# randomwons/RayTracingStudy

Measured on AMD Instinct MI355X. Metric: Mrays/s (primary+shadow) at 1920x1080, 64 spp, 100000 spheres, higher is better.
Workload: dtype f32; 1 GPU; c3: 64 spp Monte-Carlo accumulate, ~100k spheres (headline); width=1920, height=1080, spp=64, n_spheres=100000, octree_depth=7, octree_nodes=37384, prim_refs=153448, leaf_capacity=12, parallelism=single, frames_in_flight=1, rays_per_frame=184963628, primary_per_frame=132710400

## Files before the change

raytracingstudy_amd/csrc/rt_bins.h:

```cpp
#pragma once
#include <hip/hip_runtime.h>

#include "rt_bins_math.h"
#include "rt_params.h"
#include "rt_walk.h"

namespace rtamd {

typedef uint32_t bin_u32x8 __attribute__((ext_vector_type(8)));
typedef uint32_t bin_u32x2 __attribute__((ext_vector_type(2)));
typedef __attribute__((address_space(4))) const bin_u32x8 BinEntries;

struct BinBest {
    float t;
    uint32_t idx, ref;
};

__device__ __forceinline__ bool bin_entry(const bin_u32x8 e, float o0, float o1, float o2, float d0,
                                          float d1, float d2, BinBest& best) {
    if (!__any(best.t >= __uint_as_float(e[7]))) return false;
    const float4 sp = make_float4(__uint_as_float(e[0]), __uint_as_float(e[1]), __uint_as_float(e[2]),
                                  __uint_as_float(e[3]));
    float th;
    if (isect(o0, o1, o2, d0, d1, d2, sp, 0.0f, INFINITY, th)) {
        if (th < best.t || (th == best.t && e[4] < best.idx)) {
            best.t = th;
            best.idx = e[4];
            best.ref = e[5];
        }
    }
    return true;
}

__device__ __forceinline__ bool bin_nearest(uint2 hdr, unsigned long long word, bool active, float o0,
                                            float o1, float o2, float d0, float d1, float d2,
                                            float& tout, uint32_t& iout) {
    KernArgs* ka = kernargs();
    BinBest best{active ? INFINITY : -INFINITY, kNoHit, kNoHit};
    BinEntries* ent = reinterpret_cast<BinEntries*>(reinterpret_cast<uintptr_t>(ka->bin_ent)) + hdr.x;
    while (word) {
        const uint32_t k = static_cast<uint32_t>(__builtin_ctzll(word));
        word &= word - 1ull;
        if (!bin_entry(ent[k], o0, o1, o2, d0, d1, d2, best)) break;
    }
    const uint32_t nw = *reinterpret_cast<__attribute__((address_space(4))) const uint32_t*>(
        reinterpret_cast<uintptr_t>(ka->bin_info + kBinInfoWide));
    if (nw) {
        BinEntries* wide = reinterpret_cast<BinEntries*>(reinterpret_cast<uintptr_t>(ka->bin_wide));
        for (uint32_t k = 0; k < nw; ++k)
            if (!bin_entry(wide[k], o0, o1, o2, d0, d1, d2, best)) break;
    }
    if (best.ref == kNoHit) return false;
    tout = best.t;
    iout = best.ref;
    return true;
}

__device__ __forceinline__ bool bin_header(uint32_t tox, uint32_t toy, uint32_t ltw, uint32_t lth,
                                           uint2& hdr, unsigned long long& word) {
    KernArgs* ka = kernargs();
    const uint32_t flag = *reinterpret_cast<__attribute__((address_space(4))) const uint32_t*>(
        reinterpret_cast<uintptr_t>(ka->bin_info + kBinInfoFlag));
    word = 0ull;
    if (tox >= ka->W || toy >= ka->H) {
        hdr = make_uint2(0u, 0u);
        return flag != 0u;
    }
    const uint32_t b = (toy >> kBinShift) * ka->bin_nbx + (tox >> kBinShift);
    const bin_u32x2 h = *reinterpret_cast<__attribute__((address_space(4))) const bin_u32x2*>(
        reinterpret_cast<uintptr_t>(ka->bin_hdr + b));
    const size_t wi = (static_cast<size_t>(b) << (2u * kBinShift - ltw - lth)) + bin_tile_index_log2(tox, toy, ltw, lth);
    const bin_u32x2 w = *reinterpret_cast<__attribute__((address_space(4))) const bin_u32x2*>(
        reinterpret_cast<uintptr_t>(ka->bin_hdr + ka->bin_nb + wi));
    hdr = make_uint2(h.x, h.y);
    if (h.y) word = (static_cast<unsigned long long>(w.y) << 32) | w.x;
    return flag != 0u || h.y == kBinWalk;
}

}
```

raytracingstudy_amd/csrc/rt_bins_host.cpp:

```cpp
#include "rt_frame_math.h"
#include "rt_host.h"

using namespace rtamd;

namespace {

bool bins_gate(rt_renderer* r, const FrameArgs& a, const FramePlan& plan) {
    ScreenBinState& s = r->bins;
    if (r->cfg.flags & RT_FLAG_NO_BINS) return s.last_reason = RT_BINS_OFF_FLAG, false;
    if (a.count_work || !plan.inst.w8() ||
        static_cast<uint64_t>(a.W) * a.H * a.spp < s.min_samples)
        return s.last_reason = RT_BINS_OFF_KERNEL, false;
    float B[9];
    if (!bins_camera_ok(a.cam.K, a.cam.R, a.cam.o) || !cam8_basis(a.cam.K, a.cam.R, a.W, a.H, B))
        return s.last_reason = RT_BINS_OFF_CAMERA, false;
    if (bin_dense_skip_step(s.cadence, r->scene_gen, s.mirror[kBinInfoFrame], s.mirror[kBinInfoFlag]))
        return s.last_reason = RT_BINS_OFF_DENSE, false;
    return true;
}

int bins_buffers(rt_renderer* r, const FrameArgs& a, uint32_t nb, hipStream_t st) {
    ScreenBinState& s = r->bins;
    int ost;
    bool stale;
    if ((ost = s.first_ref.query(r, std::max(1u, r->n_spheres), r->scene_gen, nullptr, 0, &stale))) return ost;
    if (stale) {
        hipError_t e = launch_first_refs(a.sc.prim_sp, a.sc.prim_idx, r->prim_slots, r->d_spheres.p,
                                         r->n_spheres, s.first_ref.buf.p, st);
        if (e != hipSuccess) return hip_fail(r, e, "screen bins (first references)");
        s.first_ref.commit(r->scene_gen, nullptr, 0);
    }
    const size_t want = bin_entries_wanted(s.capacity_test, r->n_spheres, s.mirror[kBinInfoFrame],
                                           s.mirror[kBinInfoFlag], s.mirror[kBinInfoEntries],
                                           s.cadence.last_frame, s.ent.n);
    if (s.ent.n < 2 * want) {
        if (s.ent.p) RT_HIP(r, hipDeviceSynchronize());
        if ((ost = ensure(r, s.ent, 2 * want))) return ost;
    }
    if ((ost = ensure(r, s.rects, std::max(1u, r->n_spheres))) ||
        (ost = ensure(r, s.cnt, 2ull * nb + 1ull)) || (ost = ensure(r, s.offs, nb + 1ull)) ||
        (ost = ensure(r, s.hdr, size_t(nb) * (1u + kBinCap))) ||
        (ost = ensure(r, s.wide, 2ull * kBinWideCap)) || (ost = ensure(r, s.info, kBinInfoWords)))
        return ost;
    if (s.temp_items < nb + 1u || !s.temp.p) {
        const size_t bytes = bins_scan_temp_bytes(nb + 1u);
        if (!bytes) return fail(r, RT_E_HIP, "screen bins: scan scratch size");
        if ((ost = ensure(r, s.temp, bytes))) return ost;
        s.temp_items = nb + 1u;
    }
    return RT_OK;
}

BinBuild bins_build_args(const rt_renderer* r, const FrameArgs& a, const FramePlan& plan, uint32_t nbx,
                         uint32_t nby) {
    const ScreenBinState& s = r->bins;
    const uint32_t nb = nbx * nby;
    BinBuild b{};
    b.spheres = r->d_spheres.p;
    b.first_ref = s.first_ref.buf.p;
    b.n_spheres = r->n_spheres;
    memcpy(b.K, a.cam.K, sizeof(b.K));
    memcpy(b.R, a.cam.R, sizeof(b.R));
    memcpy(b.o, a.cam.o, sizeof(b.o));
    b.W = a.W;
    b.H = a.H;
    b.nbx = nbx;
    b.nby = nby;
    b.tw = plan.grid.tw;
    b.th = plan.grid.th;
    b.shrink = s.shrink;
    b.capacity = static_cast<uint32_t>(s.ent.n / 2);
    b.cap = s.cap;
    b.mean_max = s.mean_max;
    b.frame_id = a.frame_id;
    b.rects = s.rects.p;
    b.counts = s.cnt.p;
    b.cursor = s.cnt.p + nb + 1u;
    b.offs = s.offs.p;
    b.hdr = s.hdr.p;
    b.ent = s.ent.p;
    b.tiles = reinterpret_cast<unsigned long long*>(s.hdr.p + nb);
    b.wide = s.wide.p;
    b.info = s.info.p;
    b.mirror = s.mirror_dev;
    b.temp = s.temp.p;
    b.temp_bytes = s.temp.n;
    return b;
}

int bins_launch(rt_renderer* r, FrameArgs& a, const BinBuild& b, hipStream_t st) {
    ScreenBinState& s = r->bins;
    if (s.timing) RT_HIP(r, hipEventRecord(s.e0, st));
    hipError_t e = launch_screen_bins(b, st);
    if (e != hipSuccess) return hip_fail(r, e, "screen bins");
    if (s.timing) {
        RT_HIP(r, hipEventRecord(s.e1, st));
        s.timed = true;
    }
    s.last_reason = RT_BINS_ON;
    s.cadence.last_frame = a.frame_id;
    s.last_capacity = b.capacity;
    s.nbx = b.nbx;
    s.nby = b.nby;
    s.tw = b.tw;
    s.th = b.th;
    a.bin_hdr = s.hdr.p;
    a.bin_ent = s.ent.p;
    a.bin_nb = b.nbx * b.nby;
    a.bin_wide = s.wide.p;
    a.bin_info = s.info.p;
    a.bin_nbx = b.nbx;
    return RT_OK;
}

}

int rtamd::screen_bins(rt_renderer* r, FrameArgs& a, const FramePlan& plan, hipStream_t st) {
    a.bin_hdr = nullptr;
    a.bin_ent = nullptr;
    a.bin_nb = 0;
    a.bin_wide = nullptr;
    a.bin_info = nullptr;
    a.bin_nbx = 0;
    r->bins.timed = false;
    if (!bins_gate(r, a, plan)) return RT_OK;
    const uint32_t nbx = (a.W + kBinSide - 1u) / kBinSide, nby = (a.H + kBinSide - 1u) / kBinSide;
    if (const int ost = bins_buffers(r, a, nbx * nby, st)) return ost;
    return bins_launch(r, a, bins_build_args(r, a, plan, nbx, nby), st);
}

extern "C" {

int rt_get_bin_info(rt_renderer* r, rt_bin_info* info) {
// ... 71 lines not shown
```

raytracingstudy_amd/csrc/rt_bins_math.h:

```cpp
#pragma once
#include <math.h>
#include <stddef.h>
#include <stdint.h>

#if defined(__HIPCC__)
#define RT_BINS_HD __host__ __device__
#else
#define RT_BINS_HD
#endif

namespace rtamd {

constexpr uint32_t kBinShift = 3;
constexpr uint32_t kBinSide = 1u << kBinShift;
constexpr uint32_t kBinCap = 64;
constexpr uint32_t kBinWalk = 0xFFFFFFFFu;
constexpr uint32_t kBinWideCap = 32;
constexpr uint32_t kBinMeanMax = 48;
constexpr uint32_t kBinDenseSkip = 15;
constexpr uint64_t kBinMinSamples = 1ull << 22;

constexpr double kBinSlackDist = 1.0 / 131072.0;
constexpr double kBinSlackPix = 1.0 / 64.0;
constexpr double kBinSlackPixRel = 1e-6;
// ... 79 lines not shown
    return ((y & (kBinSide - 1u)) / th) * (kBinSide / tw) + (x & (kBinSide - 1u)) / tw;
}

RT_BINS_HD inline uint32_t bin_tile_index_log2(uint32_t x, uint32_t y, uint32_t ltw, uint32_t lth) {
    return (((y & (kBinSide - 1u)) >> lth) << (kBinShift - ltw)) + ((x & (kBinSide - 1u)) >> ltw);
}

RT_BINS_HD inline bool bin_rect_overlaps_tile(uint32_t rect, uint32_t tile, uint32_t tw, uint32_t th) {
    const uint32_t per_row = kBinSide / tw;
    const uint32_t tx0 = (tile % per_row) * tw, ty0 = (tile / per_row) * th;
    const uint32_t tx1 = tx0 + tw - 1u, ty1 = ty0 + th - 1u;
    return !((rect & 15u) > tx1 || ((rect >> 4) & 15u) < tx0 || ((rect >> 8) & 15u) > ty1 ||
             ((rect >> 12) & 15u) < ty0);
}

RT_BINS_HD inline uint64_t bin_tile_word(const uint32_t* rects, uint32_t cnt, uint32_t tile, uint32_t tw,
                                         uint32_t th) {
    uint64_t w = 0;
    for (uint32_t k = 0; k < cnt && k < 64u; ++k)
        if (bin_rect_overlaps_tile(rects[k], tile, tw, th)) w |= uint64_t(1) << k;
    return w;
}

enum BinInfoWord : uint32_t {
    kBinInfoFlag = 0,
    kBinInfoWide,
    kBinInfoEntries,
    kBinInfoNonEmpty,
    kBinInfoLongest,
    kBinInfoOver,
    kBinInfoFrame,
    kBinInfoWords = 8
};
constexpr uint32_t kBinFlagCapacity = 1u;
constexpr uint32_t kBinFlagWide = 2u;
constexpr uint32_t kBinFlagDense = 4u;

struct BinCadence {
    uint32_t skip = 0;
    uint64_t gen = 0;
    uint32_t last_frame = 0;
};

inline bool bin_dense_skip_step(BinCadence& c, uint64_t scene_gen, uint32_t mirror_frame,
                                uint32_t mirror_flag) {
    if (c.gen != scene_gen) c.skip = 0, c.gen = scene_gen;
    if (!c.skip && c.last_frame && mirror_frame == c.last_frame && mirror_flag == kBinFlagDense) {
        c.skip = kBinDenseSkip;
        c.last_frame = 0;
    }
    if (!c.skip) return false;
    --c.skip;
    return true;
}

inline size_t bin_entries_wanted(uint32_t capacity_test, uint32_t n_spheres, uint32_t mirror_frame,
// ... 13 lines not shown
```

raytracingstudy_amd/csrc/rt_host.h:

```cpp
#pragma once
#include <hip/hip_runtime.h>
#include <math.h>
#include <stdio.h>
#include <string.h>

#include <algorithm>
#include <chrono>
#include <string>
#include <vector>

#include "../../include/rt.h"
#include "octree_gpu.h"
#include "rt_bins_math.h"
#include "rt_overlap_math.h"
#include "rt_params.h"
#include "scene_build.h"

struct ncclComm;

namespace rtamd {

hipError_t launch_scene(const FrameArgs& a, const FramePlan& plan, hipStream_t st);
bool variant_available(uint32_t v);
hipError_t launch_compat(const FrameArgs& a, hipStream_t st);
// ... 13 lines not shown
hipError_t launch_multihit(const FrameArgs& a, const void* rays, void* hits, void* counts, uint32_t n,
                           uint32_t k, unsigned long long* counters, hipStream_t st);
hipError_t launch_overlap(const FrameArgs& a, const void* probes, void* indices, void* counts,
                          uint32_t n, uint32_t k, bool skip_self, float slack_m,
                          unsigned long long* counters, hipStream_t st);
hipError_t launch_gbuffer(const FrameArgs& a, void* hits, void* normals, void* albedo,
                          unsigned long long* counters, hipStream_t st);

struct BinBuild {
    const float4* spheres;
    const uint32_t* first_ref;
    uint32_t n_spheres;
    float K[9], R[9], o[3];
    uint32_t W, H, nbx, nby;
    uint32_t tw, th;
    double shrink;
    uint32_t capacity;
    uint32_t cap;
    uint32_t mean_max;
    uint32_t frame_id;
    uint4* rects;
    uint32_t* counts;
    uint32_t* cursor;
    uint32_t* offs;
    uint2* hdr;
    uint4* ent;
    unsigned long long* tiles;
    uint4* wide;
    uint32_t* info;
    uint32_t* mirror;
    void* temp;
    size_t temp_bytes;
};
hipError_t launch_first_refs(const float4* prim_sp, const uint32_t* prim_idx, uint32_t n_slots,
                             const float4* spheres, uint32_t n_spheres, uint32_t* first_ref,
                             hipStream_t st);
size_t bins_scan_temp_bytes(uint32_t n_items);
hipError_t launch_screen_bins(const BinBuild& b, hipStream_t st);

extern thread_local std::string g_last_error;
int fail(rt_renderer* r, int code, const std::string& msg);
int hip_fail(rt_renderer* r, hipError_t e, const char* what);

#define RT_HIP(r, call)                                   \
    do {                                                  \
        hipError_t e_ = (call);                           \
        if (e_ != hipSuccess) return hip_fail((r), e_, #call); \
    } while (0)

template <typename T>
struct DevBuf {
    T* p = nullptr;
// ... 50 lines not shown
    void* recv[F] = {nullptr, nullptr};
    std::vector<hipEvent_t> rendered[F], sent[F];
    hipEvent_t recvd[F] = {nullptr, nullptr}, unpacked[F] = {nullptr, nullptr}, out_ready = nullptr;
    bool used[F] = {false, false};
    bool timing = false;
    bool timed[F] = {false, false};
    std::vector<hipEvent_t> t_start[F], t_end[F];
    hipEvent_t t_unpacked[F] = {nullptr, nullptr};
    uint64_t frame = 0;
    bool broken = false;
    enum Fault { kNone = 0, kCreate, kComm, kSlab, kQueue };
    int fault = kNone;
    uint32_t fault_k = 0;
    uint32_t W = 0, H = 0, S = 0;
    size_t slab_bytes = 0;
    std::vector<std::vector<uint32_t>> ids;
    std::vector<uint32_t> all_ids;
    uint32_t* d_all_ids = nullptr;
};

struct ScreenBinState {
    DerivedRecords<uint32_t> first_ref;
    DevBuf<uint4> rects, ent, wide;
    DevBuf<uint32_t> cnt, offs, info;
    DevBuf<uint2> hdr;
    uint32_t tw = 1, th = 1;
    DevBuf<unsigned char> temp;
    uint32_t temp_items = 0;
    uint32_t* mirror = nullptr;
    uint32_t* mirror_dev = nullptr;
    uint32_t cap = 64, capacity_test = 0, mean_max = 48;
    double shrink = 1.0;
    uint64_t min_samples = kBinMinSamples;
    BinCadence cadence;
    uint32_t last_reason = RT_BINS_NO_FRAME;
    uint32_t last_capacity = 0, nbx = 0, nby = 0;
    hipEvent_t e0 = nullptr, e1 = nullptr;
    bool timing = false, timed = false;
    void release() {
        first_ref.buf.release();
        rects.release();
        ent.release();
        wide.release();
        cnt.release();
        offs.release();
        info.release();
        hdr.release();
        temp.release();
        if (e0) (void)hipEventDestroy(e0);
        if (e1) (void)hipEventDestroy(e1);
        if (mirror) (void)hipHostFree(mirror);
    }
};

struct QueryScratch {
    DevBuf<unsigned long long> counters;
    DevBuf<float4> ray;
    DevBuf<uint2> hit;
    DevBuf<uint2> multi_hits;
    DevBuf<uint32_t> multi_count;
    DevBuf<float4> probe;
    DevBuf<uint32_t> overlap_idx;
    DevBuf<uint32_t> overlap_count;
    void release() {
        counters.release();
        ray.release();
        hit.release();
        multi_hits.release();
        multi_count.release();
// ... 140 lines not shown
```

raytracingstudy_amd/csrc/rt_kernels.hip:

```cpp
#include <hip/hip_runtime.h>

#include <algorithm>
#include <mutex>
#include <vector>

#include "rt_params.h"
#include "rt_shade.h"
#include "rt_sorted.h"

namespace rtamd {

__device__ __forceinline__ unsigned long long wave_sum(unsigned long long v) {
#pragma unroll
    for (int off = 32; off > 0; off >>= 1) v += __shfl_xor(v, off, 64);
    return v;
}

__device__ __forceinline__ void flush_counters(const FrameArgs& a, uint32_t prim, uint32_t shadow,
                                               uint32_t nodes, uint32_t prims) {
    const unsigned long long s0 = prim;
    const unsigned long long s1 = shadow;
    const unsigned long long s2 = wave_sum(nodes);
    const unsigned long long s3 = wave_sum(prims);
    if ((threadIdx.x & 63u) == 0) {
        unsigned long long* c = a.counters + kStatLineBase + (blockIdx.x & 7u) * kStatLineStride;
        atomicAdd(c + 0, s0);
        atomicAdd(c + 1, s1);
        atomicAdd(c + 2, s2);
        atomicAdd(c + 3, s3);
    }
}

template <class C>
__device__ __forceinline__ void scene_body(FrameArgs a) {
    constexpr bool kTiles = C::tiles, kStats = C::stats, kWaveQ = C::waveq, kSort = C::sorted;
    extern __shared__ __attribute__((aligned(16))) float4 lds[];
    float4* acc = lds;
    const uint32_t wave = threadIdx.x >> 6;
    void* stk = reinterpret_cast<uint2*>(lds + (kSort ? 0u : kBlockThreads)) + threadIdx.x;
    float* wl = kSort ? reinterpret_cast<float*>(reinterpret_cast<uint2*>(lds) +
                                                 stack_levels(a.sc, true) * kBlockThreads) +
                            wave * (kSortWaveBytes / 4u)
                      : nullptr;
    const uint32_t lbs = __builtin_amdgcn_readfirstlane(leaf_buf_base(a.sc, kSort));
    if (blockIdx.x == 0) {
        KernArgs* kz = kernargs();
        for (uint32_t i = threadIdx.x; i < kz->ctr_next_words; i += kBlockThreads) kz->ctr_next[i] = 0ull;
    }
    const uint32_t tw = a.tw, th = a.th;
    uint32_t n_shadow = 0, n_nodes = 0, n_prims = 0, n_primary = 0;
#ifdef RT_BLOCK_STATS
    uint32_t bs[2 * kBlockStats] = {};
#else
    uint32_t* bs = nullptr;
#endif
#ifdef RT_TIMELINE
    const unsigned long long tl_start = wall_clock64();
    unsigned long long tl_empty = 0, tl_units = 0;
#endif
    if (kWaveQ) {
        const uint32_t gw = kTiles ? a.tile_size / tw : (a.W + tw - 1) / tw;
        const uint32_t gh = kTiles ? a.tile_size / th : (a.H + th - 1) / th;
        const uint32_t nbx = (gw + 7u) / 8u, nby = (gh + 7u) / 8u;
        const uint32_t nsx = (nbx + 7u) / 8u, nsy = (nby + 7u) / 8u;
        const uint32_t sb_grid = nsx * nsy;
        const uint32_t n_sb = kTiles ? a.n_tiles * sb_grid : sb_grid;
        const uint32_t q = blockIdx.x & 7u;
// ... 77 lines not shown
                if (kTiles) {
                    const uint32_t tile = a.tiles[k];
                    const uint32_t ts = a.tile_size;
                    tox = (tile % a.tiles_x) * ts;
                    toy = (tile / a.tiles_x) * ts;
                    obase = k * ts * ts - toy * ts - tox;
                }
            }
            for (uint32_t cur = w0; cur < w0 + chunk; ++cur) {
                const uint32_t b = cur >> 6, w = cur & 63u;
                const uint32_t wx = sx0 + (b & 7u) * 8u + (w & 7u);
                const uint32_t wy = sy0 + (b >> 3) * 8u + (w >> 3);
                if (wx >= gw || wy >= gh) continue;
                const uint32_t olx = wx * tw, oly = wy * th;
                const uint32_t ox = olx + tox, oy = oly + toy;
#ifdef RT_TIMELINE
                const unsigned long long tu0 = wall_clock64();
#endif
                if (kSort)
                    shade_pixel_sorted<C>(a, wl, stk, ox, oy, obase, n_primary, n_shadow, n_nodes,
                                          n_prims, bs);
                else
                    shade_wave_tile<C>(a, acc, stk, ox, oy, obase, n_primary, n_shadow, n_nodes,
                                       n_prims, bs, lbs);
#ifdef RT_TIMELINE
                const uint32_t sbt = k * sb_grid + (wy >> 6) * nsx + (wx >> 6);
                const unsigned long long uid = (unsigned long long)sbt * 4096u +
                                               (((wy >> 3) & 7u) * 8u + ((wx >> 3) & 7u)) * 64u +
                                               (wy & 7u) * 8u + (wx & 7u);
                if (a.timeline && (threadIdx.x & 63u) == 0 && uid < (1ull << 22)) {
                    const unsigned hw = __builtin_amdgcn_s_getreg((31 << 11) | 4);
                    const unsigned xcc = __builtin_amdgcn_s_getreg((3 << 11) | 20);
                    a.timeline[4ull * 65536 + 3 * uid] = tu0;
                    a.timeline[4ull * 65536 + 3 * uid + 1] = wall_clock64();
                    a.timeline[4ull * 65536 + 3 * uid + 2] =
                        ((unsigned long long)hw << 32) | (xcc << 16) | (blockIdx.x * 4u + wave);
                }
#endif
            }
        }
    } else {
        __shared__ uint32_t tile_slot;
        const uint32_t bts = a.bts;
        const uint32_t wtx = bts / tw, wtiles = wtx * (bts / th);
        const uint32_t per_tile = kTiles ? (a.tile_size / bts) * (a.tile_size / bts) : 0u;
        const uint32_t bx_n = (a.W + bts - 1) / bts;
        const uint32_t n_bt = kTiles ? a.n_tiles * per_tile : bx_n * ((a.H + bts - 1) / bts);
// ... 185 lines not shown
```

raytracingstudy_amd/csrc/rt_shade.h:

```cpp
#pragma once
#include <hip/hip_runtime.h>

#include "rt_params.h"
#include "rt_walk.h"
#include "rt_bins.h"

namespace rtamd {

__device__ __forceinline__ float sat(float x) { return x > 0.0f ? (x < 1.0f ? x : 1.0f) : 0.0f; }

__device__ __forceinline__ uint32_t mix32(uint32_t x) {
    x ^= x >> 16;
    x *= 0x7feb352du;
    x ^= x >> 15;
    x *= 0x846ca68bu;
    x ^= x >> 16;
    return x;
}

__device__ __forceinline__ float u01(uint32_t x) {
    return static_cast<float>(x >> 8) * (1.0f / 16777216.0f);
}

__device__ __forceinline__ void get_ray(const CamArgs& c, float u, float v, float& wx, float& wy,
// ... 8 lines not shown
    wx /= len;
    wy /= len;
    wz /= len;
}


struct PixelOut {
    float r, g, b;
};

__device__ __forceinline__ uint32_t pack_rgba8(const PixelOut& p) {
    const uint32_t r = static_cast<uint32_t>(sat(p.r) * 255.0f);
    const uint32_t g = static_cast<uint32_t>(sat(p.g) * 255.0f);
    const uint32_t b = static_cast<uint32_t>(sat(p.b) * 255.0f);
    return r | (g << 8) | (b << 16) | (255u << 24);
}

template <class C>
__device__ __forceinline__ PixelOut sample_color_unified(const FrameArgs& a, uint32_t x,
                                                         uint32_t y, uint32_t hp, uint32_t s,
                                                         bool valid, uint32_t& n_shadow,
                                                         uint32_t& n_nodes, uint32_t& n_prims,
                                                         void* stk, uint32_t* bs, uint32_t lbs,
                                                         uint32_t tox = 0, uint32_t toy = 0) {
    constexpr bool kStats = C::stats, kCam8 = C::cam8, kOcc = C::occ, kBin = C::bin;
    const SceneArgs& S = a.sc;
    KernArgs* ka = kernargs();
    float u = static_cast<float>(x), v = static_cast<float>(y);
    if (ka->jitter) {
        u = u + u01(mix32(hp ^ (s << 1)));
        v = v + u01(mix32(hp ^ ((s << 1) | 1u)));
    }
    float r0 = ka->cam.o[0], r1 = ka->cam.o[1], r2 = ka->cam.o[2];
    float d0, d1, d2;
    {
        CamArgs cam;
        for (int i = 0; i < 9; ++i) cam.K[i] = ka->cam.K[i], cam.R[i] = ka->cam.R[i];
        get_ray(cam, u, v, d0, d1, d2);
    }
    const float miss_g = sat(d1), miss_b = sat(d2);
    bool active = valid, hit0 = false;
    float lam = 0.0f;
    uint32_t al = 0;
    uint2 occ_hdr = make_uint2(0u, 0u);
#pragma unroll
    for (int phase = 0; phase < 2; ++phase) {
        float t = 0.0f;
        uint32_t idx = 0;
        bool hit = false;
        bool binned = false;
        if (kBin && phase == 0) {
            uint2 bh;
            unsigned long long bw;
            binned = !bin_header(tox, toy, static_cast<uint32_t>(__builtin_ctz(kernargs()->tw)),
                                 static_cast<uint32_t>(__builtin_ctz(kernargs()->th)), bh, bw);
            if (binned) hit = bin_nearest(bh, bw, active, r0, r1, r2, d0, d1, d2, t, idx);
        }
        if (active && !binned) {
            RT_BS(kBsPhase);
            if (phase) RT_BS(kBsPhaseShadow);
            if (phase == 0)
                hit = walk<FramePrimary<kStats, kCam8>>(S, r0, r1, r2, d0, d1, d2, 0.0f, INFINITY, t, idx,
                                                        n_nodes, n_prims, static_cast<uint2*>(stk),
                                                        false, bs, lbs);
            else if (kOcc) {
                hit = shadow_occluded<false>(S, occ_hdr, true, r0, r1, r2, static_cast<uint2*>(stk));
            } else {
                KernArgs* kl = kernargs();
                hit = walk<FrameShadow<kStats>>(
                    S, r0, r1, r2, kl->L[0], kl->L[1], kl->L[2], 0.0f, INFINITY, t, idx, n_nodes,
                    n_prims, static_cast<uint2*>(stk), true, bs);
            }
        }
        if (phase == 0) {
            hit0 = active && hit;
            bool want_shadow = false;
            KernArgs* kb = kernargs();
            if (hit0) {
                RT_BS(kBsShadeLoad);
                RT_BS(kBsShadeLoad);
                const float4 sp = kb->sc.prim_sp[idx];
                const float p0 = r0 + t * d0;
                const float p1 = r1 + t * d1;
                const float p2 = r2 + t * d2;
                const float ir = 1.0f / sp.w;
                const float n0 = (p0 - sp.x) * ir;
                const float n1 = (p1 - sp.y) * ir;
                const float n2 = (p2 - sp.z) * ir;
                const float ndl = n0 * kb->L[0] + n1 * kb->L[1] + n2 * kb->L[2];
                lam = ndl > 0.0f ? ndl : 0.0f;
                want_shadow = ndl > 0.0f && kb->shadows;
                al = kb->sc.prim_al[idx];
                if (kOcc && want_shadow) occ_hdr = kb->sc.prim_occ[idx];
                r0 = p0 + n0 * kShadowEps;
                r1 = p1 + n1 * kShadowEps;
                r2 = p2 + n2 * kShadowEps;
                d0 = kb->L[0];
                d1 = kb->L[1];
                d2 = kb->L[2];
            }
            active = want_shadow;
            n_shadow += static_cast<uint32_t>(__popcll(__ballot(active)));
            if (!__any(active)) break;
        } else if (active && hit) {
            lam = 0.0f;
        }
    }
    PixelOut c{200.0f / 255.0f, miss_g, miss_b};
    if (hit0) {
        const float amb = kernargs()->ambient;
        const float f = amb + (1.0f - amb) * lam;
        c.r = static_cast<float>(al & 0xFFu) * (1.0f / 255.0f) * f;
        c.g = static_cast<float>((al >> 8) & 0xFFu) * (1.0f / 255.0f) * f;
        c.b = static_cast<float>((al >> 16) & 0xFFu) * (1.0f / 255.0f) * f;
    }
    return c;
}

template <class C>
__device__ __forceinline__ void shade_wave_tile(const FrameArgs& a, float4* acc, void* stk,
                                                uint32_t ox, uint32_t oy, uint32_t obase,
                                                uint32_t& n_primary,
                                                uint32_t& n_shadow, uint32_t& n_nodes,
                                                uint32_t& n_prims, uint32_t* bs, uint32_t lbs) {
    constexpr bool kTiles = C::tiles, kProg = C::prog;
    const uint32_t lane = threadIdx.x & 63u;
    const uint32_t spw = a.spw, g = a.g;
    const uint32_t pix = lane / g, sub = lane & (g - 1u);
    const uint32_t qx = pix % a.tw, qy = pix / a.tw;
    const uint32_t x = ox + qx, y = oy + qy;
    const bool lane_pix = pix < a.ppw && x < a.W && y < a.H;
    const bool leader = lane_pix && sub == 0;
    const uint32_t pid = y * a.W + x;
    const uint32_t hp = mix32(a.seedmix ^ pid);
    if (kProg && a.accum_in && leader) acc[threadIdx.x] = a.accum[(size_t)y * a.W + x];
    const uint32_t s_base = kProg ? a.s_base : 0u;
    const uint32_t sub_base = s_base + sub;
    const uint32_t s_end = s_base + a.spp;
    const bool lane_ok = lane_pix && sub < spw;
    for (uint32_t r = 0; r < a.rounds; ++r) {
        const uint32_t sg = r * spw + sub_base;
        const bool valid = lane_ok && sg < s_end;
        n_primary += static_cast<uint32_t>(__popcll(__ballot(valid)));
        PixelOut c = sample_color_unified<C>(a, x, y, hp, sg, valid, n_shadow, n_nodes, n_prims, stk,
                                             bs, lbs, ox, oy);
        if (!valid) c = PixelOut{0.0f, 0.0f, 0.0f};
        for (uint32_t m = 1; m < g; m <<= 1) {
            c.r += __shfl_xor(c.r, static_cast<int>(m), 64);
            c.g += __shfl_xor(c.g, static_cast<int>(m), 64);
            c.b += __shfl_xor(c.b, static_cast<int>(m), 64);
        }
        if (leader) {
            if (r || (kProg && a.accum_in)) {
                const float4 A = acc[threadIdx.x];
                c.r = A.x + c.r;
                c.g = A.y + c.g;
                c.b = A.z + c.b;
            }
            acc[threadIdx.x] = make_float4(c.r, c.g, c.b, 0.0f);
        }
    }
    KernArgs* ko = kernargs();
    if (leader) {
        const float4 A = acc[threadIdx.x];
        if (kProg) ko->accum[(size_t)y * ko->W + x] = A;
        const float isp = ko->inv_spp;
        const PixelOut p{A.x * isp, A.y * isp, A.z * isp};
        const uint32_t rgba = pack_rgba8(p);
// ... 13 lines not shown
```

raytracingstudy_amd/csrc/rt_sorted.h:

```cpp
#pragma once
#include "rt_shade.h"

namespace rtamd {



__device__ __forceinline__ uint32_t jitter_cell(uint32_t hp, uint32_t sg) {
    const uint32_t qu = mix32(hp ^ (sg << 1)) >> (32u - kSortCellBits);
    const uint32_t qv = mix32(hp ^ ((sg << 1) | 1u)) >> (32u - kSortCellBits);
    uint32_t c = 0;
#pragma unroll
    for (uint32_t b = 0; b < kSortCellBits; ++b)
        c |= (((qu >> b) & 1u) << (2u * b)) | (((qv >> b) & 1u) << (2u * b + 1u));
    return c;
}

__device__ __forceinline__ void sample_dir(uint32_t x, uint32_t y, uint32_t hp, uint32_t sg,
                                           float& d0, float& d1, float& d2) {
    KernArgs* ka = kernargs();
    float u = static_cast<float>(x), v = static_cast<float>(y);
    if (ka->jitter) {
        u = u + u01(mix32(hp ^ (sg << 1)));
        v = v + u01(mix32(hp ^ ((sg << 1) | 1u)));
    }
// ... 62 lines not shown
    }
    for (uint32_t j = 0; j < R; ++j) {
        const uint32_t sl = 64u * j + lane;
        if (sl < n) {
            const uint32_t kp = slot[sl].x;
            ord[bcnt[kp >> 8] + (kp & 0xFFu)] = static_cast<uint8_t>(sl);
        }
    }
    uint32_t nl = 0;
    for (uint32_t r = 0; r < R; ++r) {
        const uint32_t i = 64u * r + lane;
        const bool valid = i < n;
        const uint32_t sl = valid ? static_cast<uint32_t>(ord[i]) : 0u;
        n_primary += static_cast<uint32_t>(__popcll(__ballot(valid)));
        float d0, d1, d2;
        sample_dir(x, y, hp, s_base + sl, d0, d1, d2);
        float t = 0.0f;
        uint32_t idx = 0;
        bool hit = false;
        bool binned = false;
        if (kBin) {
            uint2 bh;
            unsigned long long bw;
            binned = !bin_header(x, y, 0u, 0u, bh, bw);
            if (binned) {
                KernArgs* kc = kernargs();
                hit = bin_nearest(bh, bw, valid, kc->cam.o[0], kc->cam.o[1], kc->cam.o[2], d0, d1, d2, t,
                                  idx);
            }
        }
        if (valid && !binned) {
            RT_BS(kBsPhase);
            KernArgs* kc = kernargs();
            hit = walk<SortedPrimary<kStats>>(S, kc->cam.o[0], kc->cam.o[1], kc->cam.o[2], d0, d1, d2,
                                              0.0f, INFINITY, t, idx, n_nodes, n_prims,
                                              static_cast<uint2*>(stk), false, bs);
        }
        bool is_lit = false;
        if (valid) {
            uint2 sv = make_uint2(__float_as_uint(sat(d1)), __float_as_uint(sat(d2)));
            uint8_t kd = 0;
            if (hit) {
                const HitShade h = hit_shade(d0, d1, d2, t, idx, bs);
                is_lit = h.ndl > 0.0f && kernargs()->shadows;
                if (is_lit) {
                    sv = make_uint2(__float_as_uint(t), idx);
                    kd = 2;
                } else {
                    RT_BS(kBsShadeLoad);
                    sv = make_uint2(__float_as_uint(h.ndl > 0.0f ? h.ndl : 0.0f),
                                    kernargs()->sc.prim_al[idx]);
// ... 104 lines not shown
```

raytracingstudy_amd/csrc/screen_bins.hip:

```cpp
#include <hipcub/hipcub.hpp>

#include "rt_bins_math.h"
#include "rt_host.h"

namespace rtamd {

namespace {

__global__ void __launch_bounds__(kBlockThreads)
    first_ref_kernel(const float4* __restrict__ prim_sp, const uint32_t* __restrict__ prim_idx,
                     uint32_t n_slots, const float4* __restrict__ spheres, uint32_t n_spheres,
                     uint32_t* __restrict__ first_ref) {
    const uint32_t i = blockIdx.x * kBlockThreads + threadIdx.x;
    if (i >= n_slots) return;
    const uint32_t k = prim_idx[i];
    if (k >= n_spheres) return;
    const float4 a = prim_sp[i], b = spheres[k];
    if (__float_as_uint(a.x) != __float_as_uint(b.x) || __float_as_uint(a.y) != __float_as_uint(b.y) ||
        __float_as_uint(a.z) != __float_as_uint(b.z) || __float_as_uint(a.w) != __float_as_uint(b.w))
        return;
    atomicMin(first_ref + k, i);
}

struct BinCam {
// ... 16 lines not shown
    const uint32_t ref = first_ref[i];
    BinRect rc;
    rc.cls = kBinDropped;
    const float4 s = spheres[i];
    if (ref != kNoHit) rc = rect_of(s, cam, W, H, shrink);
    rects[i] = make_uint4(rc.x0 | (rc.x1 << 16), rc.y0 | (rc.y1 << 16), __float_as_uint(rc.near_t), rc.cls);
    if (rc.cls == kBinWide) {
        const uint32_t k = atomicAdd(info + kBinInfoWide, 1u);
        if (k < kBinWideCap) {
            wide[2u * k] = make_uint4(__float_as_uint(s.x), __float_as_uint(s.y), __float_as_uint(s.z),
                                      __float_as_uint(s.w));
            wide[2u * k + 1u] = make_uint4(i, ref, 0u | (7u << 4) | (0u << 8) | (7u << 12), __float_as_uint(rc.near_t));
        }
    } else if (rc.cls == kBinBinned) {
        for (uint32_t by = rc.y0 >> kBinShift; by <= (rc.y1 >> kBinShift); ++by)
            for (uint32_t bx = rc.x0 >> kBinShift; bx <= (rc.x1 >> kBinShift); ++bx)
                atomicAdd(counts + by * nbx + bx, 1u);
    }
}

__global__ void __launch_bounds__(kBlockThreads)
    bins_decide_kernel(const uint32_t* __restrict__ counts, const uint32_t* __restrict__ offs, uint32_t nb,
                       uint32_t capacity, uint32_t cap, uint32_t mean_max, uint32_t frame_id,
                       uint32_t* __restrict__ info, uint32_t* __restrict__ mirror) {
    __shared__ uint32_t s_ne[kBlockThreads], s_mx[kBlockThreads], s_ov[kBlockThreads];
    uint32_t ne = 0, mx = 0, ov = 0;
    for (uint32_t b = threadIdx.x; b < nb; b += kBlockThreads) {
        const uint32_t c = counts[b];
        ne += c ? 1u : 0u;
        mx = max(mx, c);
        ov += c > cap ? 1u : 0u;
    }
    s_ne[threadIdx.x] = ne;
    s_mx[threadIdx.x] = mx;
    s_ov[threadIdx.x] = ov;
    __syncthreads();
    for (uint32_t d = kBlockThreads / 2; d > 0; d >>= 1) {
        if (threadIdx.x < d) {
            s_ne[threadIdx.x] += s_ne[threadIdx.x + d];
            s_mx[threadIdx.x] = max(s_mx[threadIdx.x], s_mx[threadIdx.x + d]);
            s_ov[threadIdx.x] += s_ov[threadIdx.x + d];
        }
        __syncthreads();
    }
    if (threadIdx.x == 0) {
        const uint32_t total = offs[nb], nw = info[kBinInfoWide];
        uint32_t flag = 0u;
        if (total > capacity) flag |= kBinFlagCapacity;
        if (nw > kBinWideCap) flag |= kBinFlagWide;
        if (static_cast<unsigned long long>(total) > static_cast<unsigned long long>(mean_max) * s_ne[0])
            flag |= kBinFlagDense;
        const uint32_t w[kBinInfoWords] = {flag, nw, total, s_ne[0], s_mx[0], s_ov[0], frame_id, 0u};
        for (uint32_t k = 0; k < kBinInfoWords; ++k) {
            info[k] = w[k];
            if (k != kBinInfoFrame) __hip_atomic_store(mirror + k, w[k], __ATOMIC_RELAXED, __HIP_MEMORY_SCOPE_SYSTEM);
        }
        __hip_atomic_store(mirror + kBinInfoFrame, frame_id, __ATOMIC_RELEASE, __HIP_MEMORY_SCOPE_SYSTEM);
    }
}

__global__ void __launch_bounds__(kBlockThreads)
    bins_fill_kernel(const float4* __restrict__ spheres, const uint32_t* __restrict__ first_ref, uint32_t n,
                     const uint4* __restrict__ rects, const uint32_t* __restrict__ offs,
                     uint32_t* __restrict__ cursor, const uint32_t* __restrict__ info, uint32_t nbx,
                     uint32_t capacity, uint4* __restrict__ ent) {
    if (info[kBinInfoFlag]) return;
    const uint32_t i = blockIdx.x * kBlockThreads + threadIdx.x;
    if (i >= n) return;
    const uint4 rc = rects[i];
    if (rc.w != kBinBinned) return;
    const float4 s = spheres[i];
    const uint32_t ref = first_ref[i];
    const uint32_t x0 = rc.x & 0xFFFFu, x1 = rc.x >> 16, y0 = rc.y & 0xFFFFu, y1 = rc.y >> 16;
    const uint4 rec = make_uint4(__float_as_uint(s.x), __float_as_uint(s.y), __float_as_uint(s.z),
                                 __float_as_uint(s.w));
// ... 48 lines not shown
}

hipError_t launch_first_refs(const float4* prim_sp, const uint32_t* prim_idx, uint32_t n_slots,
                             const float4* spheres, uint32_t n_spheres, uint32_t* first_ref,
                             hipStream_t st) {
    hipError_t e = hipMemsetAsync(first_ref, 0xFF, static_cast<size_t>(n_spheres ? n_spheres : 1u) * sizeof(uint32_t), st);
    if (e != hipSuccess) return e;
    if (n_slots)
        hipLaunchKernelGGL(first_ref_kernel, dim3((n_slots + kBlockThreads - 1) / kBlockThreads),
                           dim3(kBlockThreads), 0, st, prim_sp, prim_idx, n_slots, spheres, n_spheres, first_ref);
    return hipGetLastError();
}

size_t bins_scan_temp_bytes(uint32_t n_items) {
    size_t bytes = 0;
    uint32_t* p = nullptr;
    if (hipcub::DeviceScan::ExclusiveSum(nullptr, bytes, p, p, n_items, nullptr) != hipSuccess) return 0;
    return bytes ? bytes : 1;
}

hipError_t launch_screen_bins(const BinBuild& b, hipStream_t st) {
    const uint32_t nb = b.nbx * b.nby;
    hipError_t e;
    if ((e = hipMemsetAsync(b.counts, 0, (2ull * nb + 1ull) * sizeof(uint32_t), st)) != hipSuccess) return e;
    if ((e = hipMemsetAsync(b.info, 0, kBinInfoWords * sizeof(uint32_t), st)) != hipSuccess) return e;
    BinCam cam;
    memcpy(cam.K, b.K, sizeof(cam.K));
    memcpy(cam.R, b.R, sizeof(cam.R));
    memcpy(cam.o, b.o, sizeof(cam.o));
    const uint32_t ns = (b.n_spheres + kBlockThreads - 1) / kBlockThreads;
    if (b.n_spheres)
        hipLaunchKernelGGL(bins_count_kernel, dim3(ns), dim3(kBlockThreads), 0, st, b.spheres, b.first_ref,
                           b.n_spheres, cam, b.W, b.H, b.shrink, b.nbx, b.rects, b.counts, b.info, b.wide);
    size_t bytes = b.temp_bytes;
    if ((e = hipcub::DeviceScan::ExclusiveSum(b.temp, bytes, b.counts, b.offs, nb + 1u, st)) != hipSuccess)
        return e;
    hipLaunchKernelGGL(bins_decide_kernel, dim3(1), dim3(kBlockThreads), 0, st, b.counts, b.offs, nb,
                       b.capacity, b.cap, b.mean_max, b.frame_id, b.info, b.mirror);
    if (b.n_spheres)
        hipLaunchKernelGGL(bins_fill_kernel, dim3(ns), dim3(kBlockThreads), 0, st, b.spheres, b.first_ref,
                           b.n_spheres, b.rects, b.offs, b.cursor, b.info, b.nbx, b.capacity, b.ent);
    hipLaunchKernelGGL(bins_sort_kernel, dim3((nb + kBlockThreads / 64u - 1u) / (kBlockThreads / 64u)),
                       dim3(kBlockThreads), 0, st, b.counts, b.offs, nb, b.cap, b.info, b.hdr, b.ent, b.tw,
                       b.th, bin_tiles_per_bin(b.tw, b.th), b.tiles);
    return hipGetLastError();
}

}
```

Before: 146,500 Mrays/s.

## Parallelize bin decide kernel, merge info memset, pack per-frame bin constants

Result: faster. 150,800 Mrays/s, median of 6 (+2.9%).

```diff
diff --git a/raytracingstudy_amd/csrc/rt_bins.h b/raytracingstudy_amd/csrc/rt_bins.h
--- a/raytracingstudy_amd/csrc/rt_bins.h
+++ b/raytracingstudy_amd/csrc/rt_bins.h
@@ -34,7 +34,7 @@
 
 __device__ __forceinline__ bool bin_nearest(uint2 hdr, unsigned long long word, bool active, float o0,
                                             float o1, float o2, float d0, float d1, float d2,
-                                            float& tout, uint32_t& iout) {
+                                            float& tout, uint32_t& iout, uint32_t consts) {
     KernArgs* ka = kernargs();
     BinBest best{active ? INFINITY : -INFINITY, kNoHit, kNoHit};
     BinEntries* ent = reinterpret_cast<BinEntries*>(reinterpret_cast<uintptr_t>(ka->bin_ent)) + hdr.x;
@@ -43,8 +43,7 @@
         word &= word - 1ull;
         if (!bin_entry(ent[k], o0, o1, o2, d0, d1, d2, best)) break;
     }
-    const uint32_t nw = *reinterpret_cast<__attribute__((address_space(4))) const uint32_t*>(
-        reinterpret_cast<uintptr_t>(ka->bin_info + kBinInfoWide));
+    const uint32_t nw = bin_consts_wide(consts);
     if (nw) {
         BinEntries* wide = reinterpret_cast<BinEntries*>(reinterpret_cast<uintptr_t>(ka->bin_wide));
         for (uint32_t k = 0; k < nw; ++k)
@@ -56,15 +55,21 @@
     return true;
 }
 
-__device__ __forceinline__ bool bin_header(uint32_t tox, uint32_t toy, uint32_t ltw, uint32_t lth,
-                                           uint2& hdr, unsigned long long& word) {
+__device__ __forceinline__ uint32_t bin_frame_consts(uint32_t ltw, uint32_t lth) {
+    typedef __attribute__((address_space(4))) const uint32_t ConstWord;
+    ConstWord* info = reinterpret_cast<ConstWord*>(reinterpret_cast<uintptr_t>(kernargs()->bin_info));
+    return bin_consts_pack(info[kBinInfoFlag], min(info[kBinInfoWide], kBinWideCap), ltw, lth);
+}
+
+__device__ __forceinline__ bool bin_header(uint32_t tox, uint32_t toy, uint32_t consts, uint2& hdr,
+                                           unsigned long long& word) {
     KernArgs* ka = kernargs();
-    const uint32_t flag = *reinterpret_cast<__attribute__((address_space(4))) const uint32_t*>(
-        reinterpret_cast<uintptr_t>(ka->bin_info + kBinInfoFlag));
+    const bool flag = bin_consts_flag(consts);
+    const uint32_t ltw = bin_consts_ltw(consts), lth = bin_consts_lth(consts);
     word = 0ull;
     if (tox >= ka->W || toy >= ka->H) {
         hdr = make_uint2(0u, 0u);
-        return flag != 0u;
+        return flag;
     }
     const uint32_t b = (toy >> kBinShift) * ka->bin_nbx + (tox >> kBinShift);
     const bin_u32x2 h = *reinterpret_cast<__attribute__((address_space(4))) const bin_u32x2*>(
@@ -74,7 +79,7 @@
         reinterpret_cast<uintptr_t>(ka->bin_hdr + ka->bin_nb + wi));
     hdr = make_uint2(h.x, h.y);
     if (h.y) word = (static_cast<unsigned long long>(w.y) << 32) | w.x;
-    return flag != 0u || h.y == kBinWalk;
+    return flag || h.y == kBinWalk;
 }
 
 }
diff --git a/raytracingstudy_amd/csrc/rt_bins_host.cpp b/raytracingstudy_amd/csrc/rt_bins_host.cpp
--- a/raytracingstudy_amd/csrc/rt_bins_host.cpp
+++ b/raytracingstudy_amd/csrc/rt_bins_host.cpp
@@ -38,9 +38,9 @@
         if ((ost = ensure(r, s.ent, 2 * want))) return ost;
     }
     if ((ost = ensure(r, s.rects, std::max(1u, r->n_spheres))) ||
-        (ost = ensure(r, s.cnt, 2ull * nb + 1ull)) || (ost = ensure(r, s.offs, nb + 1ull)) ||
+        (ost = ensure(r, s.cnt, bin_zeroed_words(nb))) || (ost = ensure(r, s.offs, nb + 1ull)) ||
         (ost = ensure(r, s.hdr, size_t(nb) * (1u + kBinCap))) ||
-        (ost = ensure(r, s.wide, 2ull * kBinWideCap)) || (ost = ensure(r, s.info, kBinInfoWords)))
+        (ost = ensure(r, s.wide, 2ull * kBinWideCap)))
         return ost;
     if (s.temp_items < nb + 1u || !s.temp.p) {
         const size_t bytes = bins_scan_temp_bytes(nb + 1u);
@@ -75,13 +75,14 @@
     b.frame_id = a.frame_id;
     b.rects = s.rects.p;
     b.counts = s.cnt.p;
-    b.cursor = s.cnt.p + nb + 1u;
+    b.cursor = s.cnt.p + bin_cursor_at(nb);
+    b.decide = s.cnt.p + bin_decide_at(nb);
+    b.info = s.cnt.p + bin_info_at(nb);
     b.offs = s.offs.p;
     b.hdr = s.hdr.p;
     b.ent = s.ent.p;
     b.tiles = reinterpret_cast<unsigned long long*>(s.hdr.p + nb);
     b.wide = s.wide.p;
-    b.info = s.info.p;
     b.mirror = s.mirror_dev;
     b.temp = s.temp.p;
     b.temp_bytes = s.temp.n;
@@ -108,7 +109,7 @@
     a.bin_ent = s.ent.p;
     a.bin_nb = b.nbx * b.nby;
     a.bin_wide = s.wide.p;
-    a.bin_info = s.info.p;
+    a.bin_info = b.info;
     a.bin_nbx = b.nbx;
     return RT_OK;
 }
diff --git a/raytracingstudy_amd/csrc/rt_bins_math.h b/raytracingstudy_amd/csrc/rt_bins_math.h
--- a/raytracingstudy_amd/csrc/rt_bins_math.h
+++ b/raytracingstudy_amd/csrc/rt_bins_math.h
@@ -125,6 +125,17 @@
     return w;
 }
 
+RT_BINS_HD inline bool bin_consts_fit(uint32_t wide, uint32_t ltw, uint32_t lth) {
+    return wide <= kBinWideCap && ltw <= kBinShift && lth <= kBinShift;
+}
+RT_BINS_HD inline uint32_t bin_consts_pack(uint32_t flag, uint32_t wide, uint32_t ltw, uint32_t lth) {
+    return (flag ? 1u : 0u) | (wide << 1) | (ltw << 7) | (lth << 9);
+}
+RT_BINS_HD inline bool bin_consts_flag(uint32_t c) { return (c & 1u) != 0u; }
+RT_BINS_HD inline uint32_t bin_consts_wide(uint32_t c) { return (c >> 1) & 63u; }
+RT_BINS_HD inline uint32_t bin_consts_ltw(uint32_t c) { return (c >> 7) & 3u; }
+RT_BINS_HD inline uint32_t bin_consts_lth(uint32_t c) { return (c >> 9) & 3u; }
+
 enum BinInfoWord : uint32_t {
     kBinInfoFlag = 0,
     kBinInfoWide,
@@ -135,6 +146,12 @@
     kBinInfoFrame,
     kBinInfoWords = 8
 };
+enum BinDecideWord : uint32_t { kBinDecNonEmpty = 0, kBinDecLongest, kBinDecOver, kBinDecArrived, kBinDecWords };
+inline size_t bin_cursor_at(uint32_t nb) { return size_t(nb) + 1u; }
+inline size_t bin_decide_at(uint32_t nb) { return 2u * size_t(nb) + 1u; }
+inline size_t bin_info_at(uint32_t nb) { return bin_decide_at(nb) + kBinDecWords; }
+inline size_t bin_zeroed_words(uint32_t nb) { return bin_info_at(nb) + kBinInfoWords; }
+
 constexpr uint32_t kBinFlagCapacity = 1u;
 constexpr uint32_t kBinFlagWide = 2u;
 constexpr uint32_t kBinFlagDense = 4u;
diff --git a/raytracingstudy_amd/csrc/rt_host.h b/raytracingstudy_amd/csrc/rt_host.h
--- a/raytracingstudy_amd/csrc/rt_host.h
+++ b/raytracingstudy_amd/csrc/rt_host.h
@@ -59,12 +59,13 @@
     uint4* rects;
     uint32_t* counts;
     uint32_t* cursor;
+    uint32_t* decide;
+    uint32_t* info;
     uint32_t* offs;
     uint2* hdr;
     uint4* ent;
     unsigned long long* tiles;
     uint4* wide;
-    uint32_t* info;
     uint32_t* mirror;
     void* temp;
     size_t temp_bytes;
@@ -161,7 +162,7 @@
 struct ScreenBinState {
     DerivedRecords<uint32_t> first_ref;
     DevBuf<uint4> rects, ent, wide;
-    DevBuf<uint32_t> cnt, offs, info;
+    DevBuf<uint32_t> cnt, offs;
     DevBuf<uint2> hdr;
     uint32_t tw = 1, th = 1;
     DevBuf<unsigned char> temp;
@@ -183,7 +184,6 @@
         wide.release();
         cnt.release();
         offs.release();
-        info.release();
         hdr.release();
         temp.release();
         if (e0) (void)hipEventDestroy(e0);
diff --git a/raytracingstudy_amd/csrc/rt_kernels.hip b/raytracingstudy_amd/csrc/rt_kernels.hip
--- a/raytracingstudy_amd/csrc/rt_kernels.hip
+++ b/raytracingstudy_amd/csrc/rt_kernels.hip
@@ -43,6 +43,9 @@
                             wave * (kSortWaveBytes / 4u)
                       : nullptr;
     const uint32_t lbs = __builtin_amdgcn_readfirstlane(leaf_buf_base(a.sc, kSort));
+    uint32_t binc = 0;
+    if constexpr (C::bin && !kSort)
+        binc = bin_frame_consts(static_cast<uint32_t>(__builtin_ctz(a.tw)), static_cast<uint32_t>(__builtin_ctz(a.th)));
     if (blockIdx.x == 0) {
         KernArgs* kz = kernargs();
         for (uint32_t i = threadIdx.x; i < kz->ctr_next_words; i += kBlockThreads) kz->ctr_next[i] = 0ull;
@@ -166,7 +169,7 @@
                                           n_prims, bs);
                 else
                     shade_wave_tile<C>(a, acc, stk, ox, oy, obase, n_primary, n_shadow, n_nodes,
-                                       n_prims, bs, lbs);
+                                       n_prims, bs, lbs, binc);
 #ifdef RT_TIMELINE
                 const uint32_t sbt = k * sb_grid + (wy >> 6) * nsx + (wx >> 6);
                 const unsigned long long uid = (unsigned long long)sbt * 4096u +
diff --git a/raytracingstudy_amd/csrc/rt_shade.h b/raytracingstudy_amd/csrc/rt_shade.h
--- a/raytracingstudy_amd/csrc/rt_shade.h
+++ b/raytracingstudy_amd/csrc/rt_shade.h
@@ -54,7 +54,8 @@
                                                          bool valid, uint32_t& n_shadow,
                                                          uint32_t& n_nodes, uint32_t& n_prims,
                                                          void* stk, uint32_t* bs, uint32_t lbs,
-                                                         uint32_t tox = 0, uint32_t toy = 0) {
+                                                         uint32_t tox = 0, uint32_t toy = 0,
+                                                         uint32_t binc = 0) {
     constexpr bool kStats = C::stats, kCam8 = C::cam8, kOcc = C::occ, kBin = C::bin;
     const SceneArgs& S = a.sc;
     KernArgs* ka = kernargs();
@@ -84,9 +85,8 @@
         if (kBin && phase == 0) {
             uint2 bh;
             unsigned long long bw;
-            binned = !bin_header(tox, toy, static_cast<uint32_t>(__builtin_ctz(kernargs()->tw)),
-                                 static_cast<uint32_t>(__builtin_ctz(kernargs()->th)), bh, bw);
-            if (binned) hit = bin_nearest(bh, bw, active, r0, r1, r2, d0, d1, d2, t, idx);
+            binned = !bin_header(tox, toy, binc, bh, bw);
+            if (binned) hit = bin_nearest(bh, bw, active, r0, r1, r2, d0, d1, d2, t, idx, binc);
         }
         if (active && !binned) {
             RT_BS(kBsPhase);
@@ -112,6 +112,8 @@
                 RT_BS(kBsShadeLoad);
                 RT_BS(kBsShadeLoad);
                 const float4 sp = kb->sc.prim_sp[idx];
+                al = kb->sc.prim_al[idx];
+                if (kOcc) occ_hdr = kb->sc.prim_occ[idx];
                 const float p0 = r0 + t * d0;
                 const float p1 = r1 + t * d1;
                 const float p2 = r2 + t * d2;
@@ -122,8 +124,6 @@
                 const float ndl = n0 * kb->L[0] + n1 * kb->L[1] + n2 * kb->L[2];
                 lam = ndl > 0.0f ? ndl : 0.0f;
                 want_shadow = ndl > 0.0f && kb->shadows;
-                al = kb->sc.prim_al[idx];
-                if (kOcc && want_shadow) occ_hdr = kb->sc.prim_occ[idx];
                 r0 = p0 + n0 * kShadowEps;
                 r1 = p1 + n1 * kShadowEps;
                 r2 = p2 + n2 * kShadowEps;
@@ -154,7 +154,8 @@
                                                 uint32_t ox, uint32_t oy, uint32_t obase,
                                                 uint32_t& n_primary,
                                                 uint32_t& n_shadow, uint32_t& n_nodes,
-                                                uint32_t& n_prims, uint32_t* bs, uint32_t lbs) {
+                                                uint32_t& n_prims, uint32_t* bs, uint32_t lbs,
+                                                uint32_t binc = 0) {
     constexpr bool kTiles = C::tiles, kProg = C::prog;
     const uint32_t lane = threadIdx.x & 63u;
     const uint32_t spw = a.spw, g = a.g;
@@ -175,7 +176,7 @@
         const bool valid = lane_ok && sg < s_end;
         n_primary += static_cast<uint32_t>(__popcll(__ballot(valid)));
         PixelOut c = sample_color_unified<C>(a, x, y, hp, sg, valid, n_shadow, n_nodes, n_prims, stk,
-                                             bs, lbs, ox, oy);
+                                             bs, lbs, ox, oy, binc);
         if (!valid) c = PixelOut{0.0f, 0.0f, 0.0f};
         for (uint32_t m = 1; m < g; m <<= 1) {
             c.r += __shfl_xor(c.r, static_cast<int>(m), 64);
diff --git a/raytracingstudy_amd/csrc/rt_sorted.h b/raytracingstudy_amd/csrc/rt_sorted.h
--- a/raytracingstudy_amd/csrc/rt_sorted.h
+++ b/raytracingstudy_amd/csrc/rt_sorted.h
@@ -108,11 +108,12 @@
         if (kBin) {
             uint2 bh;
             unsigned long long bw;
-            binned = !bin_header(x, y, 0u, 0u, bh, bw);
+            const uint32_t bc = bin_frame_consts(0u, 0u);
+            binned = !bin_header(x, y, bc, bh, bw);
             if (binned) {
                 KernArgs* kc = kernargs();
                 hit = bin_nearest(bh, bw, valid, kc->cam.o[0], kc->cam.o[1], kc->cam.o[2], d0, d1, d2, t,
-                                  idx);
+                                  idx, bc);
             }
         }
         if (valid && !binned) {
diff --git a/raytracingstudy_amd/csrc/screen_bins.hip b/raytracingstudy_amd/csrc/screen_bins.hip
--- a/raytracingstudy_amd/csrc/screen_bins.hip
+++ b/raytracingstudy_amd/csrc/screen_bins.hip
@@ -62,35 +62,47 @@
 __global__ void __launch_bounds__(kBlockThreads)
     bins_decide_kernel(const uint32_t* __restrict__ counts, const uint32_t* __restrict__ offs, uint32_t nb,
                        uint32_t capacity, uint32_t cap, uint32_t mean_max, uint32_t frame_id,
-                       uint32_t* __restrict__ info, uint32_t* __restrict__ mirror) {
-    __shared__ uint32_t s_ne[kBlockThreads], s_mx[kBlockThreads], s_ov[kBlockThreads];
-    uint32_t ne = 0, mx = 0, ov = 0;
-    for (uint32_t b = threadIdx.x; b < nb; b += kBlockThreads) {
-        const uint32_t c = counts[b];
-        ne += c ? 1u : 0u;
-        mx = max(mx, c);
-        ov += c > cap ? 1u : 0u;
-    }
-    s_ne[threadIdx.x] = ne;
-    s_mx[threadIdx.x] = mx;
-    s_ov[threadIdx.x] = ov;
+                       uint32_t* __restrict__ dec, uint32_t* __restrict__ info,
+                       uint32_t* __restrict__ mirror) {
+    constexpr uint32_t kWaves = kBlockThreads / 64u;
+    __shared__ uint32_t s_ne[kWaves], s_mx[kWaves], s_ov[kWaves];
+    const uint32_t b = blockIdx.x * kBlockThreads + threadIdx.x;
+    const uint32_t c = b < nb ? counts[b] : 0u;
+    uint32_t ne = c ? 1u : 0u, mx = c, ov = c > cap ? 1u : 0u;
+#pragma unroll
+    for (int off = 32; off > 0; off >>= 1) {
+        ne += __shfl_xor(ne, off, 64);
+        mx = max(mx, static_cast<uint32_t>(__shfl_xor(mx, off, 64)));
+        ov += __shfl_xor(ov, off, 64);
+    }
+    if ((threadIdx.x & 63u) == 0u) {
+        s_ne[threadIdx.x >> 6] = ne;
+        s_mx[threadIdx.x >> 6] = mx;
+        s_ov[threadIdx.x >> 6] = ov;
+    }
     __syncthreads();
-    for (uint32_t d = kBlockThreads / 2; d > 0; d >>= 1) {
-        if (threadIdx.x < d) {
-            s_ne[threadIdx.x] += s_ne[threadIdx.x + d];
-            s_mx[threadIdx.x] = max(s_mx[threadIdx.x], s_mx[threadIdx.x + d]);
-            s_ov[threadIdx.x] += s_ov[threadIdx.x + d];
-        }
-        __syncthreads();
-    }
     if (threadIdx.x == 0) {
+        for (uint32_t w = 1; w < kWaves; ++w) {
+            ne += s_ne[w];
+            mx = max(mx, s_mx[w]);
+            ov += s_ov[w];
+        }
+        if (ne) atomicAdd(dec + kBinDecNonEmpty, ne);
+        if (mx) atomicMax(dec + kBinDecLongest, mx);
+        if (ov) atomicAdd(dec + kBinDecOver, ov);
+        __threadfence();
+        if (atomicAdd(dec + kBinDecArrived, 1u) != gridDim.x - 1u) return;
+        __threadfence();
+        ne = __hip_atomic_load(dec + kBinDecNonEmpty, __ATOMIC_RELAXED, __HIP_MEMORY_SCOPE_AGENT);
+        mx = __hip_atomic_load(dec + kBinDecLongest, __ATOMIC_RELAXED, __HIP_MEMORY_SCOPE_AGENT);
+        ov = __hip_atomic_load(dec + kBinDecOver, __ATOMIC_RELAXED, __HIP_MEMORY_SCOPE_AGENT);
         const uint32_t total = offs[nb], nw = info[kBinInfoWide];
         uint32_t flag = 0u;
         if (total > capacity) flag |= kBinFlagCapacity;
         if (nw > kBinWideCap) flag |= kBinFlagWide;
-        if (static_cast<unsigned long long>(total) > static_cast<unsigned long long>(mean_max) * s_ne[0])
+        if (static_cast<unsigned long long>(total) > static_cast<unsigned long long>(mean_max) * ne)
             flag |= kBinFlagDense;
-        const uint32_t w[kBinInfoWords] = {flag, nw, total, s_ne[0], s_mx[0], s_ov[0], frame_id, 0u};
+        const uint32_t w[kBinInfoWords] = {flag, nw, total, ne, mx, ov, frame_id, 0u};
         for (uint32_t k = 0; k < kBinInfoWords; ++k) {
             info[k] = w[k];
             if (k != kBinInfoFrame) __hip_atomic_store(mirror + k, w[k], __ATOMIC_RELAXED, __HIP_MEMORY_SCOPE_SYSTEM);
@@ -185,8 +197,7 @@
 hipError_t launch_screen_bins(const BinBuild& b, hipStream_t st) {
     const uint32_t nb = b.nbx * b.nby;
     hipError_t e;
-    if ((e = hipMemsetAsync(b.counts, 0, (2ull * nb + 1ull) * sizeof(uint32_t), st)) != hipSuccess) return e;
-    if ((e = hipMemsetAsync(b.info, 0, kBinInfoWords * sizeof(uint32_t), st)) != hipSuccess) return e;
+    if ((e = hipMemsetAsync(b.counts, 0, bin_zeroed_words(nb) * sizeof(uint32_t), st)) != hipSuccess) return e;
     BinCam cam;
     memcpy(cam.K, b.K, sizeof(cam.K));
     memcpy(cam.R, b.R, sizeof(cam.R));
@@ -198,8 +209,9 @@
     size_t bytes = b.temp_bytes;
     if ((e = hipcub::DeviceScan::ExclusiveSum(b.temp, bytes, b.counts, b.offs, nb + 1u, st)) != hipSuccess)
         return e;
-    hipLaunchKernelGGL(bins_decide_kernel, dim3(1), dim3(kBlockThreads), 0, st, b.counts, b.offs, nb,
-                       b.capacity, b.cap, b.mean_max, b.frame_id, b.info, b.mirror);
+    hipLaunchKernelGGL(bins_decide_kernel, dim3((nb + kBlockThreads - 1) / kBlockThreads), dim3(kBlockThreads),
+                       0, st, b.counts, b.offs, nb, b.capacity, b.cap, b.mean_max, b.frame_id, b.decide,
+                       b.info, b.mirror);
     if (b.n_spheres)
         hipLaunchKernelGGL(bins_fill_kernel, dim3(ns), dim3(kBlockThreads), 0, st, b.spheres, b.first_ref,
                            b.n_spheres, b.rects, b.offs, b.cursor, b.info, b.nbx, b.capacity, b.ent);
```
